# ZhenlongYuan/TSAR-MVS

Hardware: AMD Instinct MI355X
Metric: depthmap Mpixels/sec (ETH3D full-res, 8 iters) (higher is better)
Workload: dtype f32

## Files before the change

include/tsar.h:

```cpp
#ifndef TSAR_H_
#define TSAR_H_

#include <stddef.h>
#include <stdint.h>

#ifdef __cplusplus
extern "C" {
#endif

#define TSAR_MAX_VIEWS 64
#define TSAR_MAXCOST 2.0f

#define TSAR_OK 0
#define TSAR_ERR_INVALID (-1)
#define TSAR_ERR_HIP (-2)
#define TSAR_ERR_STATE (-3)
#define TSAR_ERR_NOMEM (-4)

#define TSAR_MEM_HOST 0
#define TSAR_MEM_DEVICE 1

#define TSAR_COMB_ALL 0
#define TSAR_COMB_BEST_N 1
#define TSAR_COMB_ANGLE 2
// ... 62 lines not shown
int tsar_pm_iterate_final(tsar_ctx* ctx, int iters, const float* text, int mem);
int tsar_pm_cost_planes(tsar_ctx* ctx, const float* planes, int mem, float* cost_out,
                        int32_t* beview_out, float* ratio_out);
int tsar_set_plane(tsar_ctx* ctx, const float* planes, const float* cost, int mem);
int tsar_pm_sweep(tsar_ctx* ctx, int colour, int do_prop, int do_refine);
int tsar_set_sweep_counter(tsar_ctx* ctx, int n);
int tsar_get_plane(tsar_ctx* ctx, float* planes, float* cost, int32_t* beview, float* ratio, int mem);

int tsar_load_planes(tsar_ctx* ctx, const float* depth, const float* normal_world, int mem);
int tsar_compute_disp(tsar_ctx* ctx);
int tsar_compute_disp_final(tsar_ctx* ctx, const float* resize_planes, const float* text, int mem);
int tsar_depth_to_plane(tsar_ctx* ctx);

int tsar_pyramid_views(tsar_ctx* coarse, const tsar_ctx* fine);
int tsar_upsample_planes(tsar_ctx* fine, const tsar_ctx* coarse);
int tsar_compute_disp_final_upsampled(tsar_ctx* ctx, const float* text, int mem);
int tsar_get_view_image(tsar_ctx* ctx, int view, float* out, int mem);

int tsar_set_geom_depths(tsar_ctx* ctx, int n_views, const float* const* depth, int mem, float weight, float clip);
int tsar_clear_geom(tsar_ctx* ctx);
int tsar_pm_rescore(tsar_ctx* ctx);
int tsar_get_geom_matrices(tsar_ctx* ctx, int view, float* forward, float* back);

int tsar_geom_pyramid(tsar_ctx* coarse, const tsar_ctx* fine);
int tsar_pyramid_planes(tsar_ctx* coarse, const tsar_ctx* fine);
int tsar_upsample_merge(tsar_ctx* fine, const tsar_ctx* coarse);

int tsar_get_result(tsar_ctx* ctx, float* depth, float* normal_world, float* cost, float* confid,
                    int mem);

int tsar_set_reliable_mask(tsar_ctx* ctx, const float* scale, int mem);
int tsar_get_reliable_mask(tsar_ctx* ctx, float* scale, int mem);
int tsar_lrdiff(tsar_ctx* ctx);
int tsar_getview(tsar_ctx* ctx);
int tsar_wmf(tsar_ctx* ctx, int iters, int final_pass);
int tsar_set_regions(tsar_ctx* ctx, const int32_t* labels, int n_regions, const float* region_text,
                     const float* region_size, int mem);
int tsar_detect_weak_texture(tsar_ctx* ctx, int32_t* labels_out, int mem, int* n_regions_out, float* text_out,
                             float* size_out, int cap);
int tsar_ransac_regions(tsar_ctx* ctx, float* region_planes_out, float* inlier_ratio_out);
int tsar_set_region_planes(tsar_ctx* ctx, const float* region_planes);
int tsar_fake_depth(tsar_ctx* ctx, float* fakedepth_out, int mem);
int tsar_fill_textureless(tsar_ctx* ctx);

void tsar_default_slic_settings(tsar_slic_settings* s);
int tsar_slic(tsar_ctx* ctx, const uint8_t* bgra, int w, int h, const tsar_slic_settings* s,
// ... 45 lines not shown
```

tsar-mvs_amd/api.py:

```python
from __future__ import annotations

import ctypes as C
import os

import numpy as np

_HERE = os.path.dirname(os.path.abspath(__file__))
LIB_PATH = os.environ.get("TSAR_LIB") or os.path.join(_HERE, "libtsar_hip.so")

TSAR_OK = 0
TSAR_ERR_INVALID, TSAR_ERR_HIP, TSAR_ERR_STATE, TSAR_ERR_NOMEM = -1, -2, -3, -4
MEM_HOST, MEM_DEVICE = 0, 1
COMB_ALL, COMB_BEST_N, COMB_ANGLE, COMB_GOOD = 0, 1, 2, 3
FLAG_FIX_DOWN_FAR_SEED, FLAG_FIX_RIGHT_FAR_CMP, FLAG_STRICT_DIV = 1, 2, 4
FLAG_NO_LINE_CLOSING = 16
FLAG_TEX_FILTER_8BIT = 32
FLAG_FIX_INIT_RADIUS = 64
MAXCOST = 2.0
MAX_VIEWS = 64


class TsarError(RuntimeError):
    def __init__(self, code, msg):
        super().__init__(f"tsar error {code}: {msg}")
# ... 12 lines not shown

class SlicSettings(C.Structure):
    _fields_ = [("spixel_size", C.c_int32), ("no_iters", C.c_int32), ("coh_weight", C.c_float),
                ("do_enforce_connectivity", C.c_int32), ("color_space", C.c_int32)]


class FusionParams(C.Structure):
    _fields_ = [("num_consistent", C.c_int32), ("reproj_error", C.c_float), ("depth_diff", C.c_float), ("angle_deg", C.c_float),
                ("used_list", C.c_int32)]


class KernelTiming(C.Structure):
    _fields_ = [("name", C.c_char * 48), ("launches", C.c_int32), ("total_ms", C.c_float)]


SPIXEL_DTYPE = np.dtype([("center", np.float32, 2), ("color", np.float32, 4), ("id", np.int32), ("n", np.int32)])

ABI_SYMBOLS = [
    "tsar_create", "tsar_destroy", "tsar_last_error", "tsar_version", "tsar_get_stream", "tsar_synchronize",
    "tsar_default_params", "tsar_set_params", "tsar_set_views", "tsar_set_views_u8", "tsar_set_view_subset",
    "tsar_pm_init", "tsar_pm_iterate", "tsar_pm_iterate_final", "tsar_pm_sweep", "tsar_set_sweep_counter", "tsar_pm_cost_planes", "tsar_set_plane", "tsar_get_plane",
    "tsar_load_planes", "tsar_compute_disp", "tsar_compute_disp_final", "tsar_depth_to_plane", "tsar_get_result",
    "tsar_pyramid_views", "tsar_upsample_planes", "tsar_compute_disp_final_upsampled", "tsar_get_view_image",
    "tsar_set_geom_depths", "tsar_clear_geom", "tsar_pm_rescore", "tsar_get_geom_matrices",
    "tsar_geom_pyramid", "tsar_pyramid_planes", "tsar_upsample_merge",
    "tsar_set_reliable_mask", "tsar_get_reliable_mask", "tsar_lrdiff", "tsar_getview", "tsar_wmf", "tsar_set_regions", "tsar_detect_weak_texture", "tsar_ransac_regions",
    "tsar_set_region_planes", "tsar_fake_depth", "tsar_fill_textureless",
    "tsar_default_slic_settings", "tsar_slic", "tsar_default_fusion_params", "tsar_fuse", "tsar_fuse_ctx",
    "tsar_host_alloc", "tsar_host_free", "tsar_device_alloc", "tsar_device_free", "tsar_device_write", "tsar_peer_copy", "tsar_enable_kernel_timing", "tsar_reset_kernel_timing", "tsar_get_kernel_timing",
    "tsar_selftest_divide", "tsar_selftest_divide_random", "tsar_selftest_sqrt", "tsar_selftest_sweep_census", "tsar_selftest_sweep_repeat", "tsar_selftest_slic_stage",
]

_lib = None


def load_library(path: str = LIB_PATH):
    global _lib
    if _lib is not None:
        return _lib
    if not os.path.exists(path):
        raise ImportError(f"{path} not found: build it with `make -C tsar-mvs_amd/csrc` "
                          "(or __graft_entry__.build()); there is no CPU fallback")
    L = C.CDLL(path)
    L.tsar_last_error.restype = C.c_char_p
    L.tsar_last_error.argtypes = [C.c_void_p]
    L.tsar_version.restype = C.c_char_p
    L.tsar_create.argtypes = [C.c_int, C.POINTER(C.c_void_p)]
# ... 6 lines not shown
    L.tsar_set_views.argtypes = [C.c_void_p, C.c_int, C.c_int, C.c_int, C.POINTER(C.c_void_p), C.c_int, C.POINTER(Camera)]
    L.tsar_set_views_u8.argtypes = L.tsar_set_views.argtypes
    L.tsar_set_view_subset.argtypes = [C.c_void_p, C.c_int, C.c_void_p]
    L.tsar_pm_init.argtypes = [C.c_void_p]
    L.tsar_pm_iterate.argtypes = [C.c_void_p, C.c_int]
    L.tsar_pm_iterate_final.argtypes = [C.c_void_p, C.c_int, C.c_void_p, C.c_int]
    L.tsar_pm_sweep.argtypes = [C.c_void_p, C.c_int, C.c_int, C.c_int]
    L.tsar_set_sweep_counter.argtypes = [C.c_void_p, C.c_int]
    L.tsar_pm_cost_planes.argtypes = [C.c_void_p, C.c_void_p, C.c_int, C.c_void_p, C.c_void_p, C.c_void_p]
    L.tsar_set_plane.argtypes = [C.c_void_p, C.c_void_p, C.c_void_p, C.c_int]
    L.tsar_get_plane.argtypes = [C.c_void_p, C.c_void_p, C.c_void_p, C.c_void_p, C.c_void_p, C.c_int]
    L.tsar_load_planes.argtypes = [C.c_void_p, C.c_void_p, C.c_void_p, C.c_int]
    L.tsar_compute_disp.argtypes = [C.c_void_p]
    L.tsar_compute_disp_final.argtypes = [C.c_void_p, C.c_void_p, C.c_void_p, C.c_int]
    L.tsar_depth_to_plane.argtypes = [C.c_void_p]
    L.tsar_pyramid_views.argtypes = [C.c_void_p, C.c_void_p]
    L.tsar_upsample_planes.argtypes = [C.c_void_p, C.c_void_p]
    L.tsar_compute_disp_final_upsampled.argtypes = [C.c_void_p, C.c_void_p, C.c_int]
    L.tsar_get_view_image.argtypes = [C.c_void_p, C.c_int, C.c_void_p, C.c_int]
    L.tsar_set_geom_depths.argtypes = [C.c_void_p, C.c_int, C.POINTER(C.c_void_p), C.c_int, C.c_float, C.c_float]
    L.tsar_clear_geom.argtypes = [C.c_void_p]
    L.tsar_pm_rescore.argtypes = [C.c_void_p]
    L.tsar_get_geom_matrices.argtypes = [C.c_void_p, C.c_int, C.c_void_p, C.c_void_p]
    L.tsar_geom_pyramid.argtypes = [C.c_void_p, C.c_void_p]
    L.tsar_pyramid_planes.argtypes = [C.c_void_p, C.c_void_p]
    L.tsar_upsample_merge.argtypes = [C.c_void_p, C.c_void_p]
    L.tsar_get_result.argtypes = [C.c_void_p, C.c_void_p, C.c_void_p, C.c_void_p, C.c_void_p, C.c_int]
    L.tsar_set_reliable_mask.argtypes = [C.c_void_p, C.c_void_p, C.c_int]
    L.tsar_get_reliable_mask.argtypes = [C.c_void_p, C.c_void_p, C.c_int]
    L.tsar_host_alloc.restype = C.c_void_p
    L.tsar_host_alloc.argtypes = [C.c_size_t]
    L.tsar_host_free.restype = None
    L.tsar_host_free.argtypes = [C.c_void_p]
    L.tsar_device_alloc.restype = C.c_void_p
    L.tsar_device_alloc.argtypes = [C.c_int, C.c_size_t]
    L.tsar_device_free.restype = None
    L.tsar_device_free.argtypes = [C.c_int, C.c_void_p]
    L.tsar_device_write.argtypes = [C.c_int, C.c_void_p, C.c_void_p, C.c_size_t]
    L.tsar_peer_copy.argtypes = [C.c_int, C.c_void_p, C.c_int, C.c_void_p, C.c_size_t]
    L.tsar_lrdiff.argtypes = [C.c_void_p]
    L.tsar_getview.argtypes = [C.c_void_p]
    L.tsar_wmf.argtypes = [C.c_void_p, C.c_int, C.c_int]
    L.tsar_set_regions.argtypes = [C.c_void_p, C.c_void_p, C.c_int, C.c_void_p, C.c_void_p, C.c_int]
    L.tsar_detect_weak_texture.argtypes = [C.c_void_p, C.c_void_p, C.c_int, C.POINTER(C.c_int), C.c_void_p, C.c_void_p, C.c_int]
    L.tsar_ransac_regions.argtypes = [C.c_void_p, C.c_void_p, C.c_void_p]
    L.tsar_set_region_planes.argtypes = [C.c_void_p, C.c_void_p]
# ... 194 lines not shown
                continue
            if not _is_torch(d):
                d = np.ascontiguousarray(d, np.float32)
            assert tuple(d.shape) == (self.h, self.w), "depth map %d has shape %s, the views are %dx%d" % (v, tuple(d.shape), self.w, self.h)
            keep.append(d)
            p, kind = _ptr(d)
            ptrs[v] = p
            kinds.add(kind)
        assert len(kinds) <= 1, "all depth maps must live in the same memory space"
        self._chk(self.L.tsar_set_geom_depths(self._ctx, n, ptrs, kinds.pop() if kinds else MEM_HOST, float(weight), float(clip)))

    def clear_geom(self):
        self._chk(self.L.tsar_clear_geom(self._ctx))

    def rescore(self):
        self._chk(self.L.tsar_pm_rescore(self._ctx))

    def get_geom_matrices(self, view: int):
        f = np.empty((3, 4), np.float32)
        b = np.empty((3, 4), np.float32)
        self._chk(self.L.tsar_get_geom_matrices(self._ctx, view, _ptr(f)[0], _ptr(b)[0]))
        return f, b

    def geom_pyramid_from(self, fine: "Matcher"):
        self._chk(self.L.tsar_geom_pyramid(self._ctx, fine._ctx))

    def pyramid_planes_from(self, fine: "Matcher"):
        self._chk(self.L.tsar_pyramid_planes(self._ctx, fine._ctx))

    def upsample_merge(self, coarse: "Matcher"):
        self._chk(self.L.tsar_upsample_merge(self._ctx, coarse._ctx))

    def get_result(self, want=("depth", "normal", "cost", "confid"), pinned=False, out=None):
        shapes = {"depth": (self.h, self.w), "normal": (self.h, self.w, 3), "cost": (self.h, self.w), "confid": (self.h, self.w)}
        empty = pinned_empty if pinned else np.empty
        res = {}
        for k in ("depth", "normal", "cost", "confid"):
            if out is not None and k in out:
                a = out[k]
                assert a.dtype == np.float32 and tuple(a.shape) == shapes[k] and a.flags["C_CONTIGUOUS"]
                res[k] = a
            elif out is None and k in want:
                res[k] = empty(shapes[k], np.float32)
        self._chk(self.L.tsar_get_result(self._ctx, _ptr(res.get("depth"))[0], _ptr(res.get("normal"))[0], _ptr(res.get("cost"))[0],
                                         _ptr(res.get("confid"))[0], MEM_HOST))
        return res
# ... 268 lines not shown
```

tsar-mvs_amd/csrc/pm_core.h:

```cpp
#pragma once
#include <type_traits>

#include "tsar_device_math.h"

#define PM_BLOCK 256
#define PM_RW 32

typedef const uint32_t __attribute__((address_space(1)))* global_u32_ptr;
typedef const float __attribute__((address_space(1)))* global_f32_ptr;

template <bool QUAD, bool DIFF = false>
DEVFN float sample_bilinear(const DevView& vw, int w, int h, int qpitch, float u, float v, bool q8 = false) {
    u = fminf(fmaxf(u, -1.0f), (float)w);
    v = fminf(fmaxf(v, -1.0f), (float)h);
    const float fu = floorf(u), fv = floorf(v);
    float ax = u - fu, ay = v - fv;
    if (q8) { ax = rintf(ax * 256.0f) * 0.00390625f; ay = rintf(ay * 256.0f) * 0.00390625f; }
    const int iu = (int)fu, iv = (int)fv;
    float t00, t10, t01, t11;
    if (QUAD) {
        const uint32_t off = (uint32_t)(__mul24(iv + 1, qpitch) + iu + 1) * 4u;
        const uint32_t q = *(global_u32_ptr)((const char __attribute__((address_space(1)))*)vw.quad + off);
        t00 = (float)(q & 0xffu);
        t10 = (float)((q >> 8) & 0xffu);
// ... 152 lines not shown
    persp_divide_exact<true>(p0, p1, p2, xq, yq);
    const float dx = xq - xf, dy = yq - yf;
    const float e2 = dx * dx + dy * dy;
    const float tau = sc->geom_clip;
    const float r = sqrt_rsq_exact(fminf(fmaxf(e2, 0x1p-100f), 0x1p100f));
    float e = e2 < 0x1p-100f ? 0.0f : r;
    e = (inside && Dv > 0.0f && p2 > 0.0f && e2 < sc->geom_clip_sq) ? fminf(e, tau) : tau;
    return sc->geom_weight * e;
}

template <int NB, int HR, bool STRICT, bool QUAD, int V = 0, int BLK = PM_BLOCK>
DEVFN float multiview_cost(const DevScene* __restrict__ sc, const typename TileOf<QUAD>::type* tile, int tw, int own, const float* wts, const PixelRef& pr,
                           int x, int y, const float4& n4, int& beview, float& ratio) {
    constexpr bool GEOM = (V & TSAR_V_GEOM) != 0;
    constexpr int VT = V & ~(TSAR_V_GEOM | TSAR_V_REDRAW);
    float best[NB];
#pragma unroll
    for (int k = 0; k < NB; k++) best[k] = __builtin_inff();
    const int num = sc->n_sel;
    int valid = 0, bv = -1;
    float cmin = __builtin_inff();
    float depth_h = 0.0f;
    if constexpr (GEOM) depth_h = plane_depth(sc->ref, n4, x, y);
    int vi_next = sc->sel[0];
    for (int i = 0; i < num; i++) {
        const int vi = vi_next;
        vi_next = sc->sel[i + 1 < num ? i + 1 : i];
        float c;
        if constexpr ((VT & TSAR_V_LUT) != 0) c = view_cost_lut<STRICT, (VT >> 11) & 7, (VT & TSAR_V_BUF) != 0 && !STRICT, (VT & TSAR_V_MIX) != 0 && !STRICT>(sc, sc->view[vi], tile, tw, own, wts, pr, x, y, n4);
        else if constexpr (QUAD && HR == 5 && r5_production_variant(VT))
            c = view_cost_r5<STRICT, (VT & 128) != 0 && !STRICT, (VT & 8) != 0, (VT & TSAR_V_BUF) != 0, (VT & TSAR_V_MIX) != 0, BLK>(sc, sc->view[vi], tile, tw, own, wts, pr, x, y, n4);
#ifdef TSAR_EXPERIMENTS
        else if constexpr (QUAD && HR == 5 && r5_diag_variant(VT))
            c = view_cost_r5<false, true, true, true, true, BLK, (VT & 4194304) ? 1 : 2>(sc, sc->view[vi], tile, tw, own, wts, pr, x, y, n4);
#endif
        else {
            static_assert(VT == 0, "unknown tap-loop variant");
            c = view_cost_generic<HR, STRICT, QUAD, BLK>(sc, sc->view[vi], tile, tw, own, wts, pr, x, y, n4);
        }
        auto vmin = [](float a, float b) { float r; asm("v_min_f32 %0, %1, %2" : "=v"(r) : "v"(a), "v"(b)); return r; };
        auto vmax = [](float a, float b) { float r; asm("v_max_f32 %0, %1, %2" : "=v"(r) : "v"(a), "v"(b)); return r; };
        c = vmin(c, TSAR_MAXCOST);
        valid -= (int32_t)__float_as_uint(c - TSAR_MAXCOST) >> 31;
        if constexpr (GEOM) c = c + geom_term(sc, sc->view[vi], vi, x, y, depth_h);
        {
            const uint32_t worse = (uint32_t)((int32_t)__float_as_uint(cmin - c) >> 31);
            asm("v_bfi_b32 %0, %1, %2, %3" : "=v"(bv) : "v"(worse), "v"(bv), "s"(vi));
            cmin = vmin(cmin, c);
        }
        float v = c;
#pragma unroll
        for (int k = 0; k < NB; k++) {
            const float lo = vmin(best[k], v), hi = vmax(best[k], v);
            best[k] = lo;
// ... 37 lines not shown
```

tsar-mvs_amd/csrc/pm_sweep_impl.h:

```cpp
#pragma once
#include "pm_dispatch.h"

#define SWEEP_SMALL_IMAGE_TILES 3072

#define CAND_SAME (1 << 30)

DEVFN void select_candidates(const DevScene* __restrict__ sc, const float* __restrict__ c_same, const float* __restrict__ c_other,
                             int x, int y, int cand[8]) {
    const int col = sc->w, row = sc->h;
    const int p = y * col + x;
    const bool fix_seed = sc->flags & TSAR_FLAG_FIX_DOWN_FAR_SEED, fix_cmp = sc->flags & TSAR_FLAG_FIX_RIGHT_FAR_CMP;
    float cmin;
    int cp, cs;
#pragma unroll
    for (int k = 0; k < 8; k++) cand[k] = -1;
    if (y > 2) {
        cp = p - 3 * col; cmin = c_other[cp];
#pragma unroll
        for (int i = 1; i < 11; ++i)
            if (y > 2 + 2 * i) { const int q = p - (3 + 2 * i) * col; const float v = c_other[q]; if (v < cmin) { cmin = v; cp = q; } }
        cand[0] = cp;
    }
    if (y < row - 3) {
        cp = p + 3 * col;
        cmin = (fix_seed || y <= 2) ? c_other[cp] : c_other[p - 3 * col];
#pragma unroll
        for (int i = 1; i < 11; ++i)
            if (y < row - 3 - 2 * i) { const int q = p + (3 + 2 * i) * col; const float v = c_other[q]; if (v < cmin) { cmin = v; cp = q; } }
        cand[1] = cp;
    }
    if (x > 2) {
        cp = p - 3; cmin = c_other[cp];
#pragma unroll
        for (int i = 1; i < 11; ++i)
            if (x > 2 + 2 * i) { const int q = p - 3 - 2 * i; const float v = c_other[q]; if (v < cmin) { cmin = v; cp = q; } }
        cand[2] = cp;
    }
    if (x < col - 3) {
        cp = p + 3; cmin = c_other[cp];
#pragma unroll
        for (int i = 1; i < 11; ++i)
            if (x < col - 3 - 2 * i) {
                const int q = p + 3 + 2 * i;
                const float v = c_other[q];
                const bool take = fix_cmp ? (v < cmin) : (cmin < v);
                if (take) { cmin = v; cp = q; }
            }
        cand[3] = cp;
    }
    if (y > 0) {
        cp = p - col; cs = 0; cmin = c_other[cp];
#pragma unroll
        for (int i = 0; i < 3; ++i) {
            if (y > 1 + i && x > i) { const int q = p - (2 + i) * col - i; const float v = c_same[q]; if (v < cmin) { cmin = v; cp = q; cs = 1; } }
            if (y > 1 + i && x < col - 1 - i) { const int q = p - (2 + i) * col + i; const float v = c_same[q]; if (v < cmin) { cmin = v; cp = q; cs = 1; } }
        }
        cand[4] = cs ? (cp | CAND_SAME) : cp;
    }
    if (y < row - 1) {
        cp = p + col; cs = 0; cmin = c_other[cp];
#pragma unroll
        for (int i = 0; i < 3; ++i) {
            if (y < row - 2 - i && x > i) { const int q = p + (2 + i) * col - i; const float v = c_same[q]; if (v < cmin) { cmin = v; cp = q; cs = 1; } }
            if (y < row - 2 - i && x < col - 1 - i) { const int q = p + (2 + i) * col + i; const float v = c_same[q]; if (v < cmin) { cmin = v; cp = q; cs = 1; } }
        }
        cand[5] = cs ? (cp | CAND_SAME) : cp;
    }
    if (x > 0) {
        cp = p - 1; cs = 0; cmin = c_other[cp];
#pragma unroll
        for (int i = 0; i < 3; ++i) {
            if (x > 1 + i && y > i) { const int q = p - (2 + i) - i * col; const float v = c_same[q]; if (v < cmin) { cmin = v; cp = q; cs = 1; } }
            if (x > 1 + i && y < row - 1 - i) { const int q = p - (2 + i) + i * col; const float v = c_same[q]; if (v < cmin) { cmin = v; cp = q; cs = 1; } }
        }
        cand[6] = cs ? (cp | CAND_SAME) : cp;
    }
    if (x < col - 1) {
        cp = p + 1; cs = 0; cmin = c_other[cp];
#pragma unroll
        for (int i = 0; i < 3; ++i) {
            if (x < col - 2 - i && y > i) { const int q = p + (2 + i) - i * col; const float v = c_same[q]; if (v < cmin) { cmin = v; cp = q; cs = 1; } }
            if (x < col - 2 - i && y < row - 1 - i) { const int q = p + (2 + i) + i * col; const float v = c_same[q]; if (v < cmin) { cmin = v; cp = q; cs = 1; } }
        }
        cand[7] = cs ? (cp | CAND_SAME) : cp;
    }
}

DEVFN bool same_bits(const float4& a, const float4& b) {
    return __float_as_uint(a.x) == __float_as_uint(b.x) && __float_as_uint(a.y) == __float_as_uint(b.y) &&
           __float_as_uint(a.z) == __float_as_uint(b.z) && __float_as_uint(a.w) == __float_as_uint(b.w);
}

struct SweepMemo {
    int32_t* cand;
    uint32_t* seq;
    uint32_t* changed;
    uint32_t launch, valid_from;
    int mode;
    int slot_off;
};

template <int NB, int HR, bool STRICT, bool QUAD, int V = 0, int BLK = PM_BLOCK, bool CMP = false>
__global__ __launch_bounds__(BLK) void pm_sweep_kernel(const DevScene* __restrict__ sc, int colour,
                                                            const float* __restrict__ c_same, const float4* __restrict__ n_same,
                                                            const float* __restrict__ c_other, const float4* __restrict__ n_other,
                                                            float* c_out, float4* n_out, float* __restrict__ ratio_out,
                                                            int32_t* __restrict__ beview_out, uint32_t stream_id, int do_prop,
// ... 47 lines not shown
    float ratio_w = 0.f;
    int beview_w = 0;
    const DevRef& rf = sc->ref;
    const bool work = mine && pr.textured;
    int cand[8] = {-1, -1, -1, -1, -1, -1, -1, -1};
    if (work && do_prop) {
        select_candidates(sc, c_same, c_other, x, y, cand);
        if (memo.mode) {
            const uint32_t m_seq = memo.seq[p];
            const bool have = m_seq >= memo.valid_from && cost_consistent;
            const int4* mc = (const int4*)(memo.cand + (size_t)p * 8);
            int prev[8];
            if (have) {
                const int4 a0 = mc[0], a1 = mc[1];
                prev[0] = a0.x; prev[1] = a0.y; prev[2] = a0.z; prev[3] = a0.w; prev[4] = a1.x; prev[5] = a1.y; prev[6] = a1.z; prev[7] = a1.w;
            }
            int4 w0, w1;
            w0.x = cand[0]; w0.y = cand[1]; w0.z = cand[2]; w0.w = cand[3]; w1.x = cand[4]; w1.y = cand[5]; w1.z = cand[6]; w1.w = cand[7];
            ((int4*)(memo.cand + (size_t)p * 8))[0] = w0;
            ((int4*)(memo.cand + (size_t)p * 8))[1] = w1;
            memo.seq[p] = memo.launch;
            if (have) {
#pragma unroll
                for (int a = 0; a < 8; a++)
                    if (cand[a] >= 0 && cand[a] == prev[a] && memo.changed[cand[a] & 0x3fffffff] < m_seq) cand[a] = -1;
            }
        }
    }
    float depth_now = 0.f;
    float vv[3] = {0.f, 0.f, 0.f};
    if (work) { depth_now = plane_depth(rf, n_now, x, y); view_vector(rf, x, y, vv); }
    const float4 n_first = n_now;
    float deltaN = 1.0f;
    float deltaZ = sc->max_disp / 2.0f;
    const float fb = rf.f * rf.baseline;
    const int n_ref = do_refine ? sc->refine_steps : 0;

    if constexpr (!CMP) {
        if (work) {
            const int h_end = 8 + n_ref;
#pragma unroll 1
            for (int h = do_prop ? 0 : 8; h < h_end; h++) {
                float4 n_t;
                float depth_t;
                if (h < 8) {
                    int ci = cand[0];
#pragma unroll
                    for (int a = 1; a < 8; a++) ci = (h == a) ? cand[a] : ci;
// ... 240 lines not shown
```

tsar-mvs_amd/csrc/pm_tap_r5.h:

```cpp
#pragma once

template <bool STRICT, bool ROW, bool D16, bool BUF, bool MIX, int BLK, int DIAG = 0>
DEVFN float view_cost_r5(const DevScene* __restrict__ sc, const DevView& vw, const unsigned short* tile, int tw, int own, const float* wts,
                         const PixelRef& pr, int x, int y, const float4& n4) {
    static_assert(!(STRICT && ROW), "the row-wise walk changes the summation order: fast mode only");
    static_assert(!MIX || (BUF && !STRICT), "the half-float difference texture serves the fast arithmetic's blend through buffer loads");
    const int w = sc->w, h = sc->h, qp = sc->quad_pitch;
    const int qorg = (qp + 1) << 2;
    float H[9];
    if (STRICT) plane_homography(sc->ref, vw, n4, H, sc->k_sparse != 0);
    else plane_homography_fast(sc->ref, vw, n4, H);
    float sum_src = 0.f, sum_src_src = 0.f, sum_ref_src = 0.f;
    bool need_clamp;
    if (!STRICT) {
        const float xc = (float)x, yc = (float)y;
        const float Xc = fma_(H[1], yc, fma_(H[0], xc, H[2])), Yc = fma_(H[4], yc, fma_(H[3], xc, H[5])), Zc = fma_(H[7], yc, fma_(H[6], xc, H[8]));
        const float a = fabsf(H[0]) + fabsf(H[1]), b = fabsf(H[3]) + fabsf(H[4]), c = fabsf(H[6]) + fabsf(H[7]);
        const float Zmin = fma_(-5.0f, c, Zc);
        const float r = __builtin_amdgcn_rcpf(Zmin * Zc);
        const float r5 = 5.0f * r, rc = Zmin * r;
        const float du = fma_(a, Zc, fabsf(Xc) * c) * r5, dv = fma_(b, Zc, fabsf(Yc) * c) * r5;
        const float uc = Xc * rc, vc = Yc * rc;
        const bool inside = Zmin > 0.0f && fminf(uc - du, vc - dv) >= 1.5f && uc + du <= (float)(w - 1) - 1.5f && vc + dv <= (float)(h - 1) - 1.5f;
        need_clamp = !__all(inside);
    } else {
        bool inside = true;
        float zmin = __builtin_inff(), zmax = 0.0f;
#pragma unroll
        for (int c = 0; c < 4; c++) {
            const float xi = (float)(x + ((c & 1) ? 5 : -5)), yj = (float)(y + ((c & 2) ? 5 : -5));
            const float X = fma_(H[1], yj, fma_(H[0], xi, H[2])), Y = fma_(H[4], yj, fma_(H[3], xi, H[5])), Z = fma_(H[7], yj, fma_(H[6], xi, H[8]));
            const float rz = __builtin_amdgcn_rcpf(Z);
            const float u = X * rz, v = Y * rz;
            inside = inside && Z > 0.0f && u >= 1.0f && u <= (float)(w - 1) - 1.0f && v >= 1.0f && v <= (float)(h - 1) - 1.0f;
            if (STRICT) { zmin = fminf(zmin, Z); zmax = fmaxf(zmax, Z); }
        }
        if (STRICT) {
            const float cm = (float)(max(w, h) + 32);
            const float sz = fma_(fabsf(H[6]) + fabsf(H[7]), cm, fabsf(H[8]));
            const float sx = fma_(fabsf(H[0]) + fabsf(H[1]), cm, fabsf(H[2]));
            const float sy = fma_(fabsf(H[3]) + fabsf(H[4]), cm, fabsf(H[5]));
            inside = inside && zmin >= 3.814697265625e-06f && zmax <= 131072.0f && sz * cm <= 524288.0f * zmin && fmaxf(sx, sy) <= 262144.0f * zmin;
        }
        need_clamp = !__all(inside);
    }
    uint32_t qb_lo = 0, qb_hi = 0;
    if (!BUF) {
        const uint64_t qa = (uint64_t)(uintptr_t)vw.quad + (uint32_t)qorg;
        qb_lo = __builtin_amdgcn_readfirstlane((uint32_t)qa);
        qb_hi = __builtin_amdgcn_readfirstlane((uint32_t)(qa >> 32));
        asm volatile("" : "+s"(qb_lo), "+s"(qb_hi));
    }
    typedef uint32_t u32x4s __attribute__((ext_vector_type(4)));
    u32x4s rsrc = {0u, 0u, 0u, 0u};
    if (BUF) {
        if (MIX) {
            const uint64_t da = (uint64_t)(uintptr_t)vw.dquad + 2 * (uint64_t)(uint32_t)qorg;
            rsrc.x = __builtin_amdgcn_readfirstlane((uint32_t)da);
            rsrc.y = __builtin_amdgcn_readfirstlane(((uint32_t)(da >> 32) & 0xffffu) | (8u << 16));
        } else {
        const uint64_t qa = (uint64_t)(uintptr_t)vw.quad + (uint32_t)qorg;
        rsrc.x = __builtin_amdgcn_readfirstlane((uint32_t)qa);
        rsrc.y = __builtin_amdgcn_readfirstlane(((uint32_t)(qa >> 32) & 0xffffu) | (4u << 16));
        }
        rsrc.z = __builtin_amdgcn_readfirstlane((uint32_t)(qp * (h + 1) - 1));
        rsrc.w = 0x00020000u;
        asm volatile("" : "+s"(rsrc));
    }
    typedef float f32x2 __attribute__((ext_vector_type(2)));
    auto line6 = [&](int i, auto clamp_tag, auto unr_tag) {
        constexpr bool CLAMP = decltype(clamp_tag)::value;
        constexpr bool UNR = decltype(unr_tag)::value;
        static_assert(!UNR || (ROW && D16), "the unrolled form is written for the row-wise walk with D16 window loads");
        const float xi = (float)((ROW ? y : x) + i);
        const float bx = STRICT ? H[0] * xi : fma_(H[ROW ? 1 : 0], xi, H[2]), by = STRICT ? H[3] * xi : fma_(H[ROW ? 4 : 3], xi, H[5]),
                    bz = STRICT ? H[6] * xi : fma_(H[ROW ? 7 : 6], xi, H[8]);
        const int line = (i + 5) >> 1;
        float rcol[6];
        f32x2 wcol[3];
        {
            constexpr int U = BLK / 64, S = ROW ? 6 : 1;
            const uint32_t wa = (uint32_t)(uintptr_t)(const __attribute__((address_space(3))) float*)(wts + (UNR ? 0 : (ROW ? line : 6 * line) * BLK));
#pragma unroll
            for (int k = 0; k < 3; k++)
                asm("ds_read2st64_b32 %0, %1 offset0:%2 offset1:%3" : "=v"(wcol[k]) : "v"(wa), "n"(2 * U * S * k + (UNR ? U * line : 0)), "n"(2 * U * S * k + U * S + (UNR ? U * line : 0)), "v"(bz));
        }
        if (D16) {
            const uint32_t a0 = (uint32_t)(uintptr_t)(const __attribute__((address_space(3))) unsigned short*)(UNR ? tile + own - 5 * tw - 5 : ROW ? tile + own + i * tw - 5 : tile + own + i - 5 * tw);
#pragma unroll
            for (int jj = 0; jj < 6; jj++)
// ... 136 lines not shown
```

tsar-mvs_amd/csrc/tsar_api.hip:

```cpp
#include <math.h>
#include <stdio.h>
#include <stdlib.h>
#include <string.h>

#include <algorithm>

#include "tsar_dev.h"

ScopedKernelTimer::ScopedKernelTimer(tsar_ctx* c, const char* name) : ctx(c) {
    if (!ctx->timing || !name) return;
    for (size_t k = 0; k < ctx->timers.size(); k++)
        if (ctx->timers[k].name == name) ti = (int)k;
    if (ti < 0) {
        ctx->timers.emplace_back();
        ctx->timers.back().name = name;
        ti = (int)ctx->timers.size() - 1;
    }
    if (hipEventCreate(&e0) != hipSuccess) { ti = -1; return; }
    if (hipEventCreate(&e1) != hipSuccess) { hipEventDestroy(e0); ti = -1; return; }
    hipEventRecord(e0, ctx->stream);
}
ScopedKernelTimer::~ScopedKernelTimer() {
    if (ti < 0) return;
    hipEventRecord(e1, ctx->stream);
// ... 174 lines not shown
    sc.n_best = p.n_best;
    sc.cost_comb = p.cost_comb;
    sc.flags = p.flags;
    sc.seed_lo = (uint32_t)p.seed;
    sc.seed_hi = (uint32_t)(p.seed >> 32);
    sc.lut_row_major = (p.flags & TSAR_FLAG_STRICT_DIV) ? 0 : 1;
    std::vector<int> d2;
    for (int i = -sc.hrad; i <= sc.hrad; i += 2)
        for (int j = -sc.vrad; j <= sc.vrad; j += 2) d2.push_back(i * i + j * j);
    std::sort(d2.begin(), d2.end());
    d2.erase(std::unique(d2.begin(), d2.end()), d2.end());
    sc.lut_classes = (int)d2.size() <= TSAR_LUT_MAX_CLASSES ? (int)d2.size() : 0;
    for (int k = 0; k < sc.lut_classes; k++) sc.lut_d2[k] = d2[k];
    const int rl = sc.lut_row_major ? sc.vrad : sc.hrad, rt = sc.lut_row_major ? sc.hrad : sc.vrad;
    sc.lut_chunk = lut_chunk_taps(rt + 1);
    sc.lut_pad_taps = (rt + sc.lut_chunk) / sc.lut_chunk * sc.lut_chunk;
    for (uint32_t& r : sc.tap_row) r = (uint32_t)sc.lut_classes * 1024u;
    for (int l = 0; l <= rl && sc.lut_classes; l++)
        for (int t = 0; t <= rt; t++) {
            const int a = 2 * l - rl, b = 2 * t - rt;
            sc.tap_row[l * sc.lut_pad_taps + t] = 1024u * (uint32_t)(std::lower_bound(d2.begin(), d2.end(), a * a + b * b) - d2.begin());
        }
}
static int upload_scene(tsar_ctx* ctx) {
    if (!ctx->dscene) TRY(dev_alloc(ctx, &ctx->dscene, 1));
    TSAR_HIP_TRY(ctx, hipMemcpyAsync(ctx->dscene, &ctx->hscene, sizeof(DevScene), hipMemcpyHostToDevice, ctx->stream));
    TSAR_HIP_TRY(ctx, hipStreamSynchronize(ctx->stream));
    return TSAR_OK;
}

extern "C" const char* tsar_version(void) {
#ifdef TSAR_EXPERIMENTS
    return "tsar-mvs_amd 0.2.0 (gfx950) +experiments";
#else
    return "tsar-mvs_amd 0.2.0 (gfx950)";
#endif
}

static void read_knobs(tsar_ctx* ctx) {
    auto num = [](const char* name, int dflt) { const char* e = getenv(name); return e && e[0] ? atoi(e) : dflt; };
    auto on = [](const char* name, bool dflt) { const char* e = getenv(name); return e && e[0] ? e[0] != '0' : dflt; };
    ctx->variant = num("TSAR_VARIANT", ctx->variant);
    ctx->buffer_gather = on("TSAR_BUFFER_GATHER", true);
    ctx->mix_gather = on("TSAR_MIX_GATHER", true);
    ctx->strip_w = num("TSAR_STRIP", -1);
    ctx->buffer_from = num("TSAR_BUFFER_FROM", 1);
    ctx->force_block = num("TSAR_BLOCK", 0);
    ctx->memo_mode = num("TSAR_MEMO", 1);
// ... 612 lines not shown
    TRY(launch_pm_rescore(ctx, ctx->buf[0].n4, ctx->buf[1].c, ctx->buf[1].n4, ctx->beview, ctx->ratio));
    TSAR_HIP_TRY(ctx, hipStreamSynchronize(ctx->stream));
    std::swap(ctx->buf[0], ctx->buf[1]);
    ctx->sweeps_done = 0;
    ctx->cost_consistent = true;
    ctx->memo_valid_from = ctx->launch_seq + 1;
    ctx->have_out = false;
    return TSAR_OK;
}

extern "C" int tsar_get_geom_matrices(tsar_ctx* ctx, int view, float* forward, float* back) {
    CHECK_CTX(ctx);
    NEED_VIEWS(ctx);
    if (view < 0 || view >= ctx->n_views || !forward || !back) return fail(ctx, TSAR_ERR_INVALID, "tsar_get_geom_matrices: view out of range or NULL output");
    const DevView& dv = ctx->hscene.view[view];
    for (int r = 0; r < 3; r++) {
        for (int c = 0; c < 3; c++) forward[4 * r + c] = dv.A[3 * r + c];
        forward[4 * r + 3] = dv.b[r];
    }
    for (int i = 0; i < 12; i++) back[i] = ctx->hscene.geom_back[view][i];
    return TSAR_OK;
}

static bool is_pyramid_of(const tsar_ctx* coarse, const tsar_ctx* fine) {
    if (!coarse->have_views || !fine->have_views || coarse->device != fine->device) return false;
    if (coarse->w != (fine->w + 1) / 2 || coarse->h != (fine->h + 1) / 2 || coarse->n_views != fine->n_views) return false;
    if (coarse->cams.size() != fine->cams.size()) return false;
    for (size_t v = 0; v < fine->cams.size(); v++) {
        tsar_camera c = fine->cams[v];
        c.K[0] *= 0.5f; c.K[2] *= 0.5f; c.K[4] *= 0.5f; c.K[5] *= 0.5f;
        if (memcmp(&c, &coarse->cams[v], sizeof c) != 0) return false;
    }
    return true;
}

extern "C" int tsar_geom_pyramid(tsar_ctx* coarse, const tsar_ctx* fine_in) {
    CHECK_CTX(coarse);
    tsar_ctx* fine = const_cast<tsar_ctx*>(fine_in);
    if (!fine || fine == coarse) return fail(coarse, TSAR_ERR_INVALID, "tsar_geom_pyramid: fine must be another context");
    if (!fine->hscene.geom_on) return fail(coarse, TSAR_ERR_STATE, "tsar_geom_pyramid: the fine context has no geometric-consistency term");
    if (!is_pyramid_of(coarse, fine))
        return fail(coarse, TSAR_ERR_INVALID, "tsar_geom_pyramid: the coarse context must hold fine's views one level down (tsar_pyramid_views)");
    TSAR_HIP_TRY(coarse, hipStreamSynchronize(coarse->stream));
    free_geom(coarse);
    const size_t np = (size_t)coarse->w * coarse->h;
    coarse->geom_maps.assign(coarse->n_views, nullptr);
// ... 340 lines not shown
```

tsar-mvs_amd/csrc/tsar_dev.h:

```cpp
#pragma once
#include <hip/hip_runtime.h>
#include <stdint.h>
#include <stdlib.h>

#include <string>
#include <vector>

#include "../../include/tsar.h"

#define TSAR_LUT_LINES 32
#define TSAR_LUT_TAPS 40
#define TSAR_LUT_MAX_CLASSES 144
#define TSAR_MAX_SELECTED 32

struct DevView {
    float K[9];
    float R[9];
    float t[3];
    float t_abs_lo;
    float A[9];
    float b[3];
    float t_abs_hi;
    const float* img;
    const uint32_t* quad;
    const uint2* dquad;
};

struct DevRef {
    float K[9];
    float Kinv[9];
    float Minv[9];
    float Rorig[9];
    float RorigInv[9];
    float P34[3];
    float C[3];
    float fx, f, alpha, baseline, depthMin, depthMax;
};

struct DevScene {
    int w, h;
    int n_sel;
    int hrad, vrad;
    int n_best, cost_comb;
    int refine_steps;
    int quad_pitch;
    int use_quad;
    float min_disp, max_disp;
    uint32_t flags;
    uint32_t seed_lo, seed_hi;
    int k_sparse;
    DevRef ref;
    int sel[TSAR_MAX_VIEWS];
    DevView view[TSAR_MAX_VIEWS];
    int lut_classes;
    int lut_row_major;
    int lut_chunk;
    int lut_pad_taps;
    int lut_d2[TSAR_LUT_MAX_CLASSES];
    uint32_t tap_row[TSAR_LUT_LINES * TSAR_LUT_TAPS + 8];
    const float* geom_depth[TSAR_MAX_VIEWS];
    float geom_back[TSAR_MAX_VIEWS][12];
    float geom_weight, geom_clip, geom_clip_sq;
    int geom_on;
};

#define TSAR_V_LUT 1024
#define TSAR_V_BUF 131072
#define TSAR_V_MIX 2097152
#define TSAR_V_GEOM 16777216
#define TSAR_V_REDRAW 33554432

struct PlaneBuf {
    float* c;
    float4* n4;
};

struct KernelTimer {
    std::string name;
    int launches = 0;
    float total_ms = 0.f;
    std::vector<std::pair<hipEvent_t, hipEvent_t>> pending;
};

struct ScratchArena {
    char* base = nullptr;
    size_t cap = 0;
// ... 156 lines not shown
```

Measured before the change: 47.27.

## Pipeline per-view camera and buffer-descriptor loads via packed 128-byte view blocks

Adds a host-precomputed, 128-byte-aligned per-view block holding the matrix, translation, buffer resource descriptors and view index, so each view is read from one contiguous line. The r5 cost loop prefetches the next view's block while the current view is evaluated, and builds the homography from scalar-register camera values and a per-pixel hoisted Kinv*n/d term. Candidate selection and the memo check are also rewritten as branchless min/bfi sequences in inline asm. A debug readback API is added. The cost is more live registers for the prefetched block and a larger scene struct.

Measured after the change: 46.64. 1.3% lower.

```diff
diff --git a/include/tsar.h b/include/tsar.h
--- a/include/tsar.h
+++ b/include/tsar.h
@@ -108,6 +108,8 @@
 int tsar_pm_rescore(tsar_ctx* ctx);
 int tsar_get_geom_matrices(tsar_ctx* ctx, int view, float* forward, float* back);
 
+int tsar_debug_read_view_blocks(tsar_ctx* ctx, uint32_t* fast_out, uint32_t* view_out, int32_t* sel_out, int32_t* dims);
+
 int tsar_geom_pyramid(tsar_ctx* coarse, const tsar_ctx* fine);
 int tsar_pyramid_planes(tsar_ctx* coarse, const tsar_ctx* fine);
 int tsar_upsample_merge(tsar_ctx* fine, const tsar_ctx* coarse);
diff --git a/tsar-mvs_amd/api.py b/tsar-mvs_amd/api.py
--- a/tsar-mvs_amd/api.py
+++ b/tsar-mvs_amd/api.py
@@ -58,7 +58,7 @@
     "tsar_pm_init", "tsar_pm_iterate", "tsar_pm_iterate_final", "tsar_pm_sweep", "tsar_set_sweep_counter", "tsar_pm_cost_planes", "tsar_set_plane", "tsar_get_plane",
     "tsar_load_planes", "tsar_compute_disp", "tsar_compute_disp_final", "tsar_depth_to_plane", "tsar_get_result",
     "tsar_pyramid_views", "tsar_upsample_planes", "tsar_compute_disp_final_upsampled", "tsar_get_view_image",
-    "tsar_set_geom_depths", "tsar_clear_geom", "tsar_pm_rescore", "tsar_get_geom_matrices",
+    "tsar_set_geom_depths", "tsar_clear_geom", "tsar_pm_rescore", "tsar_get_geom_matrices", "tsar_debug_read_view_blocks",
     "tsar_geom_pyramid", "tsar_pyramid_planes", "tsar_upsample_merge",
     "tsar_set_reliable_mask", "tsar_get_reliable_mask", "tsar_lrdiff", "tsar_getview", "tsar_wmf", "tsar_set_regions", "tsar_detect_weak_texture", "tsar_ransac_regions",
     "tsar_set_region_planes", "tsar_fake_depth", "tsar_fill_textureless",
@@ -111,6 +111,7 @@
     L.tsar_clear_geom.argtypes = [C.c_void_p]
     L.tsar_pm_rescore.argtypes = [C.c_void_p]
     L.tsar_get_geom_matrices.argtypes = [C.c_void_p, C.c_int, C.c_void_p, C.c_void_p]
+    L.tsar_debug_read_view_blocks.argtypes = [C.c_void_p, C.c_void_p, C.c_void_p, C.c_void_p, C.c_void_p]
     L.tsar_geom_pyramid.argtypes = [C.c_void_p, C.c_void_p]
     L.tsar_pyramid_planes.argtypes = [C.c_void_p, C.c_void_p]
     L.tsar_upsample_merge.argtypes = [C.c_void_p, C.c_void_p]
@@ -351,6 +352,15 @@
         self._chk(self.L.tsar_get_geom_matrices(self._ctx, view, _ptr(f)[0], _ptr(b)[0]))
         return f, b
 
+    def read_view_blocks(self):
+        fast = np.zeros((32, 32), np.uint32)
+        view = np.zeros((32, 16), np.uint32)
+        sel = np.zeros(32, np.int32)
+        dims = np.zeros(4, np.int32)
+        self._chk(self.L.tsar_debug_read_view_blocks(self._ctx, _ptr(fast)[0], _ptr(view)[0], _ptr(sel)[0], _ptr(dims)[0]))
+        n = int(dims[3])
+        return fast[:n], view[:n], sel[:n], dims
+
     def geom_pyramid_from(self, fine: "Matcher"):
         self._chk(self.L.tsar_geom_pyramid(self._ctx, fine._ctx))
 
diff --git a/tsar-mvs_amd/csrc/pm_core.h b/tsar-mvs_amd/csrc/pm_core.h
--- a/tsar-mvs_amd/csrc/pm_core.h
+++ b/tsar-mvs_amd/csrc/pm_core.h
@@ -198,14 +198,29 @@
     float cmin = __builtin_inff();
     float depth_h = 0.0f;
     if constexpr (GEOM) depth_h = plane_depth(sc->ref, n4, x, y);
-    int vi_next = sc->sel[0];
+    constexpr bool PIPE = !STRICT && QUAD && HR == 5 && (VT & TSAR_V_LUT) == 0 && r5_production_variant(VT);
+    constexpr bool PBUF = (VT & TSAR_V_BUF) != 0, PMIX = (VT & TSAR_V_MIX) != 0;
+    ViewPipe vp;
+    int vi_next = 0;
+    if constexpr (PIPE) {
+        view_pipe_load<PBUF, PMIX>(vp, &sc->fast[0]);
+        const float inv_d = __builtin_amdgcn_rcpf(n4.w);
+#pragma unroll
+        for (int c = 0; c < 3; c++) vp.m[c] = fma_(n4.z, sc->ref.Kinv[6 + c], fma_(n4.y, sc->ref.Kinv[3 + c], n4.x * sc->ref.Kinv[c])) * inv_d;
+    } else vi_next = sc->sel[0];
     for (int i = 0; i < num; i++) {
-        const int vi = vi_next;
-        vi_next = sc->sel[i + 1 < num ? i + 1 : i];
+        int vi;
+        if constexpr (PIPE) {
+            vi = vp.vi;
+            vp.next = i + 1 < num ? i + 1 : i;
+        } else {
+            vi = vi_next;
+            vi_next = sc->sel[i + 1 < num ? i + 1 : i];
+        }
         float c;
         if constexpr ((VT & TSAR_V_LUT) != 0) c = view_cost_lut<STRICT, (VT >> 11) & 7, (VT & TSAR_V_BUF) != 0 && !STRICT, (VT & TSAR_V_MIX) != 0 && !STRICT>(sc, sc->view[vi], tile, tw, own, wts, pr, x, y, n4);
         else if constexpr (QUAD && HR == 5 && r5_production_variant(VT))
-            c = view_cost_r5<STRICT, (VT & 128) != 0 && !STRICT, (VT & 8) != 0, (VT & TSAR_V_BUF) != 0, (VT & TSAR_V_MIX) != 0, BLK>(sc, sc->view[vi], tile, tw, own, wts, pr, x, y, n4);
+            c = view_cost_r5<STRICT, (VT & 128) != 0 && !STRICT, (VT & 8) != 0, (VT & TSAR_V_BUF) != 0, (VT & TSAR_V_MIX) != 0, BLK, 0, PIPE>(sc, sc->view[vi], tile, tw, own, wts, pr, x, y, n4, &vp);
 #ifdef TSAR_EXPERIMENTS
         else if constexpr (QUAD && HR == 5 && r5_diag_variant(VT))
             c = view_cost_r5<false, true, true, true, true, BLK, (VT & 4194304) ? 1 : 2>(sc, sc->view[vi], tile, tw, own, wts, pr, x, y, n4);
diff --git a/tsar-mvs_amd/csrc/pm_sweep_impl.h b/tsar-mvs_amd/csrc/pm_sweep_impl.h
--- a/tsar-mvs_amd/csrc/pm_sweep_impl.h
+++ b/tsar-mvs_amd/csrc/pm_sweep_impl.h
@@ -4,6 +4,18 @@
 #define SWEEP_SMALL_IMAGE_TILES 3072
 
 #define CAND_SAME (1 << 30)
+
+DEVFN uint32_t take_if_less(float v, int q, float& cmin, int& cp) {
+    const uint32_t taken = (uint32_t)((int32_t)__float_as_uint(v - cmin) >> 31);
+    asm("v_bfi_b32 %0, %1, %2, %3" : "=v"(cp) : "v"(taken), "v"(q), "v"(cp));
+    asm("v_min_f32 %0, %1, %2" : "=v"(cmin) : "v"(cmin), "v"(v));
+    return taken;
+}
+DEVFN void take_if_greater(float v, int q, float& cmin, int& cp) {
+    const uint32_t taken = (uint32_t)((int32_t)__float_as_uint(cmin - v) >> 31);
+    asm("v_bfi_b32 %0, %1, %2, %3" : "=v"(cp) : "v"(taken), "v"(q), "v"(cp));
+    asm("v_max_f32 %0, %1, %2" : "=v"(cmin) : "v"(cmin), "v"(v));
+}
 
 DEVFN void select_candidates(const DevScene* __restrict__ sc, const float* __restrict__ c_same, const float* __restrict__ c_other,
                              int x, int y, int cand[8]) {
@@ -11,14 +23,15 @@
     const int p = y * col + x;
     const bool fix_seed = sc->flags & TSAR_FLAG_FIX_DOWN_FAR_SEED, fix_cmp = sc->flags & TSAR_FLAG_FIX_RIGHT_FAR_CMP;
     float cmin;
-    int cp, cs;
+    int cp;
+    uint32_t cs;
 #pragma unroll
     for (int k = 0; k < 8; k++) cand[k] = -1;
     if (y > 2) {
         cp = p - 3 * col; cmin = c_other[cp];
 #pragma unroll
         for (int i = 1; i < 11; ++i)
-            if (y > 2 + 2 * i) { const int q = p - (3 + 2 * i) * col; const float v = c_other[q]; if (v < cmin) { cmin = v; cp = q; } }
+            if (y > 2 + 2 * i) { const int q = p - (3 + 2 * i) * col; take_if_less(c_other[q], q, cmin, cp); }
         cand[0] = cp;
     }
     if (y < row - 3) {
@@ -26,14 +39,14 @@
         cmin = (fix_seed || y <= 2) ? c_other[cp] : c_other[p - 3 * col];
 #pragma unroll
         for (int i = 1; i < 11; ++i)
-            if (y < row - 3 - 2 * i) { const int q = p + (3 + 2 * i) * col; const float v = c_other[q]; if (v < cmin) { cmin = v; cp = q; } }
+            if (y < row - 3 - 2 * i) { const int q = p + (3 + 2 * i) * col; take_if_less(c_other[q], q, cmin, cp); }
         cand[1] = cp;
     }
     if (x > 2) {
         cp = p - 3; cmin = c_other[cp];
 #pragma unroll
         for (int i = 1; i < 11; ++i)
-            if (x > 2 + 2 * i) { const int q = p - 3 - 2 * i; const float v = c_other[q]; if (v < cmin) { cmin = v; cp = q; } }
+            if (x > 2 + 2 * i) { const int q = p - 3 - 2 * i; take_if_less(c_other[q], q, cmin, cp); }
         cand[2] = cp;
     }
     if (x < col - 3) {
@@ -43,8 +56,8 @@
             if (x < col - 3 - 2 * i) {
                 const int q = p + 3 + 2 * i;
                 const float v = c_other[q];
-                const bool take = fix_cmp ? (v < cmin) : (cmin < v);
-                if (take) { cmin = v; cp = q; }
+                if (fix_cmp) take_if_less(v, q, cmin, cp);
+                else take_if_greater(v, q, cmin, cp);
             }
         cand[3] = cp;
     }
@@ -52,37 +65,37 @@
         cp = p - col; cs = 0; cmin = c_other[cp];
 #pragma unroll
         for (int i = 0; i < 3; ++i) {
-            if (y > 1 + i && x > i) { const int q = p - (2 + i) * col - i; const float v = c_same[q]; if (v < cmin) { cmin = v; cp = q; cs = 1; } }
-            if (y > 1 + i && x < col - 1 - i) { const int q = p - (2 + i) * col + i; const float v = c_same[q]; if (v < cmin) { cmin = v; cp = q; cs = 1; } }
-        }
-        cand[4] = cs ? (cp | CAND_SAME) : cp;
+            if (y > 1 + i && x > i) { const int q = p - (2 + i) * col - i; cs |= take_if_less(c_same[q], q, cmin, cp); }
+            if (y > 1 + i && x < col - 1 - i) { const int q = p - (2 + i) * col + i; cs |= take_if_less(c_same[q], q, cmin, cp); }
+        }
+        cand[4] = cp | (int)(cs & CAND_SAME);
     }
     if (y < row - 1) {
         cp = p + col; cs = 0; cmin = c_other[cp];
 #pragma unroll
         for (int i = 0; i < 3; ++i) {
-            if (y < row - 2 - i && x > i) { const int q = p + (2 + i) * col - i; const float v = c_same[q]; if (v < cmin) { cmin = v; cp = q; cs = 1; } }
-            if (y < row - 2 - i && x < col - 1 - i) { const int q = p + (2 + i) * col + i; const float v = c_same[q]; if (v < cmin) { cmin = v; cp = q; cs = 1; } }
-        }
-        cand[5] = cs ? (cp | CAND_SAME) : cp;
+            if (y < row - 2 - i && x > i) { const int q = p + (2 + i) * col - i; cs |= take_if_less(c_same[q], q, cmin, cp); }
+            if (y < row - 2 - i && x < col - 1 - i) { const int q = p + (2 + i) * col + i; cs |= take_if_less(c_same[q], q, cmin, cp); }
+        }
+        cand[5] = cp | (int)(cs & CAND_SAME);
     }
     if (x > 0) {
         cp = p - 1; cs = 0; cmin = c_other[cp];
 #pragma unroll
         for (int i = 0; i < 3; ++i) {
-            if (x > 1 + i && y > i) { const int q = p - (2 + i) - i * col; const float v = c_same[q]; if (v < cmin) { cmin = v; cp = q; cs = 1; } }
-            if (x > 1 + i && y < row - 1 - i) { const int q = p - (2 + i) + i * col; const float v = c_same[q]; if (v < cmin) { cmin = v; cp = q; cs = 1; } }
-        }
-        cand[6] = cs ? (cp | CAND_SAME) : cp;
+            if (x > 1 + i && y > i) { const int q = p - (2 + i) - i * col; cs |= take_if_less(c_same[q], q, cmin, cp); }
+            if (x > 1 + i && y < row - 1 - i) { const int q = p - (2 + i) + i * col; cs |= take_if_less(c_same[q], q, cmin, cp); }
+        }
+        cand[6] = cp | (int)(cs & CAND_SAME);
     }
     if (x < col - 1) {
         cp = p + 1; cs = 0; cmin = c_other[cp];
 #pragma unroll
         for (int i = 0; i < 3; ++i) {
-            if (x < col - 2 - i && y > i) { const int q = p + (2 + i) - i * col; const float v = c_same[q]; if (v < cmin) { cmin = v; cp = q; cs = 1; } }
-            if (x < col - 2 - i && y < row - 1 - i) { const int q = p + (2 + i) + i * col; const float v = c_same[q]; if (v < cmin) { cmin = v; cp = q; cs = 1; } }
-        }
-        cand[7] = cs ? (cp | CAND_SAME) : cp;
+            if (x < col - 2 - i && y > i) { const int q = p + (2 + i) - i * col; cs |= take_if_less(c_same[q], q, cmin, cp); }
+            if (x < col - 2 - i && y < row - 1 - i) { const int q = p + (2 + i) + i * col; cs |= take_if_less(c_same[q], q, cmin, cp); }
+        }
+        cand[7] = cp | (int)(cs & CAND_SAME);
     }
 }
 
@@ -176,8 +189,9 @@
             memo.seq[p] = memo.launch;
             if (have) {
 #pragma unroll
-                for (int a = 0; a < 8; a++)
-                    if (cand[a] >= 0 && cand[a] == prev[a] && memo.changed[cand[a] & 0x3fffffff] < m_seq) cand[a] = -1;
+                for (int a = 0; a < 8; a++) {
+                    if (cand[a] >= 0 && cand[a] == prev[a]) cand[a] |= (int32_t)(memo.changed[cand[a] & 0x3fffffff] - m_seq) >> 31;
+                }
             }
         }
     }
diff --git a/tsar-mvs_amd/csrc/pm_tap_r5.h b/tsar-mvs_amd/csrc/pm_tap_r5.h
--- a/tsar-mvs_amd/csrc/pm_tap_r5.h
+++ b/tsar-mvs_amd/csrc/pm_tap_r5.h
@@ -1,14 +1,49 @@
 #pragma once
 
-template <bool STRICT, bool ROW, bool D16, bool BUF, bool MIX, int BLK, int DIAG = 0>
+typedef uint32_t u32x4s __attribute__((ext_vector_type(4)));
+struct ViewPipe {
+    float cam[12];
+    u32x4s rs;
+    uint32_t qlo, qhi;
+    int vi;
+    float m[3];
+    int next;
+};
+template <bool BUF, bool MIX>
+DEVFN void view_pipe_load(ViewPipe& vp, const DevViewFast* __restrict__ f) {
+#pragma unroll
+    for (int k = 0; k < 9; k++) vp.cam[k] = f->A[k];
+#pragma unroll
+    for (int k = 0; k < 3; k++) vp.cam[9 + k] = f->b[k];
+    if (BUF) {
+        const uint32_t* r = MIX ? f->rsrc_dquad : f->rsrc_quad;
+        vp.rs.x = r[0]; vp.rs.y = r[1]; vp.rs.z = r[2]; vp.rs.w = r[3];
+    } else {
+        vp.qlo = f->quad_lo; vp.qhi = f->quad_hi;
+    }
+    vp.vi = f->vi;
+}
+
+template <bool STRICT, bool ROW, bool D16, bool BUF, bool MIX, int BLK, int DIAG = 0, bool PIPE = false>
 DEVFN float view_cost_r5(const DevScene* __restrict__ sc, const DevView& vw, const unsigned short* tile, int tw, int own, const float* wts,
-                         const PixelRef& pr, int x, int y, const float4& n4) {
+                         const PixelRef& pr, int x, int y, const float4& n4, ViewPipe* vp = nullptr) {
     static_assert(!(STRICT && ROW), "the row-wise walk changes the summation order: fast mode only");
+    static_assert(!PIPE || !STRICT, "the pipelined view block serves the fast arithmetic's homography");
     static_assert(!MIX || (BUF && !STRICT), "the half-float difference texture serves the fast arithmetic's blend through buffer loads");
     const int w = sc->w, h = sc->h, qp = sc->quad_pitch;
     const int qorg = (qp + 1) << 2;
     float H[9];
     if (STRICT) plane_homography(sc->ref, vw, n4, H, sc->k_sparse != 0);
+    else if (PIPE) {
+#pragma unroll
+        for (int k = 0; k < 12; k++) vp->cam[k] = __int_as_float(__builtin_amdgcn_readfirstlane(__float_as_int(vp->cam[k])));
+        asm volatile("" : "+s"(vp->cam[0]), "+s"(vp->cam[1]), "+s"(vp->cam[2]), "+s"(vp->cam[3]), "+s"(vp->cam[4]), "+s"(vp->cam[5]),
+                          "+s"(vp->cam[6]), "+s"(vp->cam[7]), "+s"(vp->cam[8]), "+s"(vp->cam[9]), "+s"(vp->cam[10]), "+s"(vp->cam[11]));
+#pragma unroll
+        for (int r = 0; r < 3; r++)
+#pragma unroll
+            for (int c = 0; c < 3; c++) H[r * 3 + c] = fma_(-vp->cam[9 + r], vp->m[c], vp->cam[r * 3 + c]);
+    }
     else plane_homography_fast(sc->ref, vw, n4, H);
     float sum_src = 0.f, sum_src_src = 0.f, sum_ref_src = 0.f;
     bool need_clamp;
@@ -45,15 +80,21 @@
         need_clamp = !__all(inside);
     }
     uint32_t qb_lo = 0, qb_hi = 0;
-    if (!BUF) {
+    if (PIPE && !BUF) {
+        qb_lo = __builtin_amdgcn_readfirstlane(vp->qlo); qb_hi = __builtin_amdgcn_readfirstlane(vp->qhi);
+        asm volatile("" : "+s"(qb_lo), "+s"(qb_hi));
+    } else if (!BUF) {
         const uint64_t qa = (uint64_t)(uintptr_t)vw.quad + (uint32_t)qorg;
         qb_lo = __builtin_amdgcn_readfirstlane((uint32_t)qa);
         qb_hi = __builtin_amdgcn_readfirstlane((uint32_t)(qa >> 32));
         asm volatile("" : "+s"(qb_lo), "+s"(qb_hi));
     }
-    typedef uint32_t u32x4s __attribute__((ext_vector_type(4)));
     u32x4s rsrc = {0u, 0u, 0u, 0u};
-    if (BUF) {
+    if (PIPE && BUF) {
+        rsrc.x = __builtin_amdgcn_readfirstlane(vp->rs.x); rsrc.y = __builtin_amdgcn_readfirstlane(vp->rs.y);
+        rsrc.z = __builtin_amdgcn_readfirstlane(vp->rs.z); rsrc.w = __builtin_amdgcn_readfirstlane(vp->rs.w);
+        asm volatile("" : "+s"(rsrc));
+    } else if (BUF) {
         if (MIX) {
             const uint64_t da = (uint64_t)(uintptr_t)vw.dquad + 2 * (uint64_t)(uint32_t)qorg;
             rsrc.x = __builtin_amdgcn_readfirstlane((uint32_t)da);
@@ -66,6 +107,11 @@
         rsrc.z = __builtin_amdgcn_readfirstlane((uint32_t)(qp * (h + 1) - 1));
         rsrc.w = 0x00020000u;
         asm volatile("" : "+s"(rsrc));
+    }
+    if (PIPE) {
+        int nx = __builtin_amdgcn_readfirstlane(vp->next);
+        asm volatile("" : "+s"(nx));
+        view_pipe_load<BUF, MIX>(*vp, &sc->fast[nx]);
     }
     typedef float f32x2 __attribute__((ext_vector_type(2)));
     auto line6 = [&](int i, auto clamp_tag, auto unr_tag) {
diff --git a/tsar-mvs_amd/csrc/tsar_api.hip b/tsar-mvs_amd/csrc/tsar_api.hip
--- a/tsar-mvs_amd/csrc/tsar_api.hip
+++ b/tsar-mvs_amd/csrc/tsar_api.hip
@@ -220,8 +220,38 @@
             sc.tap_row[l * sc.lut_pad_taps + t] = 1024u * (uint32_t)(std::lower_bound(d2.begin(), d2.end(), a * a + b * b) - d2.begin());
         }
 }
+static void fill_fast_views(DevScene& sc) {
+    const uint32_t qorg = (uint32_t)(sc.quad_pitch + 1) << 2;
+    const uint32_t records = (uint32_t)(sc.quad_pitch * (sc.h + 1) - 1);
+    for (int i = 0; i < TSAR_MAX_VIEWS; i++) {
+        DevViewFast& f = sc.fast[i];
+        memset(&f, 0, sizeof f);
+        if (i >= sc.n_sel) continue;
+        const DevView& v = sc.view[sc.sel[i]];
+        memcpy(f.A, v.A, sizeof f.A);
+        memcpy(f.b, v.b, sizeof f.b);
+        f.vi = sc.sel[i];
+        if (v.quad) {
+            const uint64_t qa = (uint64_t)(uintptr_t)v.quad + qorg;
+            f.quad_lo = (uint32_t)qa;
+            f.quad_hi = (uint32_t)(qa >> 32);
+            f.rsrc_quad[0] = (uint32_t)qa;
+            f.rsrc_quad[1] = ((uint32_t)(qa >> 32) & 0xffffu) | (4u << 16);
+            f.rsrc_quad[2] = records;
+            f.rsrc_quad[3] = 0x00020000u;
+        }
+        if (v.dquad) {
+            const uint64_t da = (uint64_t)(uintptr_t)v.dquad + 2 * (uint64_t)qorg;
+            f.rsrc_dquad[0] = (uint32_t)da;
+            f.rsrc_dquad[1] = ((uint32_t)(da >> 32) & 0xffffu) | (8u << 16);
+            f.rsrc_dquad[2] = records;
+            f.rsrc_dquad[3] = 0x00020000u;
+        }
+    }
+}
 static int upload_scene(tsar_ctx* ctx) {
     if (!ctx->dscene) TRY(dev_alloc(ctx, &ctx->dscene, 1));
+    fill_fast_views(ctx->hscene);
     TSAR_HIP_TRY(ctx, hipMemcpyAsync(ctx->dscene, &ctx->hscene, sizeof(DevScene), hipMemcpyHostToDevice, ctx->stream));
     TSAR_HIP_TRY(ctx, hipStreamSynchronize(ctx->stream));
     return TSAR_OK;
@@ -880,6 +910,27 @@
     return TSAR_OK;
 }
 
+extern "C" int tsar_debug_read_view_blocks(tsar_ctx* ctx, uint32_t* fast_out, uint32_t* view_out, int32_t* sel_out, int32_t* dims) {
+    CHECK_CTX(ctx);
+    NEED_VIEWS(ctx);
+    if (!fast_out || !view_out || !sel_out || !dims) return fail(ctx, TSAR_ERR_INVALID, "tsar_debug_read_view_blocks: NULL output");
+    std::vector<unsigned char> raw(sizeof(DevScene) + 128);
+    DevScene* d = (DevScene*)(((uintptr_t)raw.data() + 127) & ~(uintptr_t)127);
+    TSAR_HIP_TRY(ctx, hipMemcpy((void*)d, ctx->dscene, sizeof(DevScene), hipMemcpyDeviceToHost));
+    dims[0] = d->w; dims[1] = d->h; dims[2] = d->quad_pitch; dims[3] = d->n_sel;
+    for (int i = 0; i < d->n_sel && i < TSAR_MAX_VIEWS; i++) {
+        memcpy(fast_out + 32 * i, &d->fast[i], 128);
+        const DevView& v = d->view[d->sel[i]];
+        uint32_t* o = view_out + 16 * i;
+        memcpy(o, v.A, 36);
+        memcpy(o + 9, v.b, 12);
+        const uint64_t qa = (uint64_t)(uintptr_t)v.quad, da = (uint64_t)(uintptr_t)v.dquad;
+        o[12] = (uint32_t)qa; o[13] = (uint32_t)(qa >> 32); o[14] = (uint32_t)da; o[15] = (uint32_t)(da >> 32);
+        sel_out[i] = d->sel[i];
+    }
+    return TSAR_OK;
+}
+
 static bool is_pyramid_of(const tsar_ctx* coarse, const tsar_ctx* fine) {
     if (!coarse->have_views || !fine->have_views || coarse->device != fine->device) return false;
     if (coarse->w != (fine->w + 1) / 2 || coarse->h != (fine->h + 1) / 2 || coarse->n_views != fine->n_views) return false;
diff --git a/tsar-mvs_amd/csrc/tsar_dev.h b/tsar-mvs_amd/csrc/tsar_dev.h
--- a/tsar-mvs_amd/csrc/tsar_dev.h
+++ b/tsar-mvs_amd/csrc/tsar_dev.h
@@ -36,6 +36,17 @@
     float C[3];
     float fx, f, alpha, baseline, depthMin, depthMax;
 };
+
+struct alignas(128) DevViewFast {
+    float A[9];
+    float b[3];
+    uint32_t rsrc_quad[4];
+    uint32_t rsrc_dquad[4];
+    uint32_t quad_lo, quad_hi;
+    int vi;
+    int pad[5];
+};
+static_assert(sizeof(DevViewFast) == 128, "one view block per 128-byte line");
 
 struct DevScene {
     int w, h;
@@ -62,6 +73,7 @@
     float geom_back[TSAR_MAX_VIEWS][12];
     float geom_weight, geom_clip, geom_clip_sq;
     int geom_on;
+    DevViewFast fast[TSAR_MAX_VIEWS];
 };
 
 #define TSAR_V_LUT 1024
```
